# rhoposit/self-attention-tacotron

Hardware: AMD Instinct MI355X
Metric: teacher-forced mel frames/sec, LJSpeech batch=32, 1/2/4/8 MI355X (higher is better)
Workload: dtype fp32; 1 GPU; LJSpeech self-attention-tacotron.json teacher-forced training step (fwd + BPTT + Adam), configs[1]; global_batch=32, per_gpu_batch=32, chars=200, mel_frames=1000, num_mels=80, r=2, decoder_steps=500, parallelism=dp1, hip_graph=True, params=6227928

## Files before the change

include/sat_abi.h:

```cpp
#ifndef SAT_ABI_H
#define SAT_ABI_H

#include <stdint.h>

#ifdef __cplusplus
extern "C" {
#endif

#define SAT_OK 0
#define SAT_ERR_ARGUMENT -1
#define SAT_ERR_HIP -2
#define SAT_ERR_UNSUPPORTED -3

#define SAT_ABI_VERSION 11

int sat_version(void);
int sat_abi_version(void);
const char* sat_last_error_string(void);
int sat_device_arch(char* buf, int len);

typedef struct SatGemmDesc {
  int32_t M, N, K, batch;
  int32_t a_mode, a_L, a_C, a_shift;
  const float* A;
  int64_t a_sm, a_sk, a_sbatch;
  int32_t b_mode, b_taps, b_C, act;
  const float* B;
  int64_t b_sk, b_sn, b_sbatch;
  float* C;
// ... 288 lines not shown

typedef struct SatDecAttnFwd {
  int32_t B, N, T, U, M1, M2, D1, D2, F, KW;
  float u, zc, zh;
  const float* X0; const float* W0r; const float* Wq1; const float* Wq2;
  const float* K1; const float* V1; const float* K2; const float* V2;
  const int64_t* lengths;
  const float* v1; const float* b1; const float* convW; const float* convb; const float* locW;
  const float* v2;
  const float* mask_c; const float* mask_h;
  float* REC0; float* C0; float* H0RAW; float* G0; float* Q;
  float* S1; float* AL1; float* S2; float* ST; float* LOC;
  float* E; float* PART; float* QP; uint32_t* ctr; int32_t* err;
  int64_t* prof;
  float* ZH;
} SatDecAttnFwd;

int sat_decoder_attention_fwd(const SatDecAttnFwd* args, void* stream);
int64_t sat_decoder_attention_scratch(int32_t B, int32_t N, int64_t* e_floats, int64_t* part_floats,
                                      int64_t* qp_floats);

typedef struct SatDecAttnBwd {
  int32_t B, N, T, U, M1, M2, D1, D2, F, KW;
  float u, zc, zh;
  const float* REC0; const float* C0; const float* G0;
  const float* S1; const float* AL1; const float* S2; const float* ST; const float* LOC;
  const float* V1; const float* V2;
  const float* v1; const float* convW; const float* convb; const float* locW;
  const float* v2;
  const float* W0r; const float* Wq1; const float* Wq2;
// ... 199 lines not shown
```

self-attention-tacotron_amd/_lib.py:

```python

from __future__ import annotations

import ctypes
import os
from typing import Optional

PKG_DIR = os.path.dirname(os.path.abspath(__file__))
LIB_PATH = os.environ.get("SAT_LIB_OVERRIDE") or os.path.join(PKG_DIR, "libsat_hip.so")


class SatLibraryError(RuntimeError):

    def __init__(self, msg: str, rc: Optional[int] = None):
        super().__init__(msg)
        self.rc = rc


SAT_ERR_ARGUMENT = -1
SAT_ERR_UNSUPPORTED = -3


class SatGemmDesc(ctypes.Structure):
    _fields_ = [
        ("M", ctypes.c_int32), ("N", ctypes.c_int32), ("K", ctypes.c_int32),
# ... 91 lines not shown
SatAttnAgentBwd = _struct("SatAttnAgentBwd", """
    i32:B i32:ntiles i32:M1 i32:D1 i32:D2 ptr:dup ptr:u_t ptr:agent_w ptr:dz_out
    ptr:dctx i64:dctx_sb ptr:dq_extra i64:dq_sb""")

SatAttnParamGrad = _struct("SatAttnParamGrad", """
    i32:T i32:B i32:N i32:D1 i32:D2 i32:F i32:KW i32:att1_forward ptr:K1 ptr:K2
    ptr:q i64:q_tstride i64:q_bstride ptr:b1 ptr:v1 ptr:locW ptr:v2 ptr:loc
    ptr:s_prev i64:s_tstride ptr:de1 ptr:de2 ptr:df ptr:dK1 ptr:dK2 ptr:pg i64:pg_stride
    i32:tsplit""")

SatDecAttnFwd = _struct("SatDecAttnFwd", """
    i32:B i32:N i32:T i32:U i32:M1 i32:M2 i32:D1 i32:D2 i32:F i32:KW f32:u f32:zc f32:zh
    ptr:X0 ptr:W0r ptr:Wq1 ptr:Wq2 ptr:K1 ptr:V1 ptr:K2 ptr:V2 ptr:lengths
    ptr:v1 ptr:b1 ptr:convW ptr:convb ptr:locW ptr:v2 ptr:mask_c ptr:mask_h
    ptr:REC0 ptr:C0 ptr:H0RAW ptr:G0 ptr:Q ptr:S1 ptr:AL1 ptr:S2 ptr:ST ptr:LOC
    ptr:E ptr:PART ptr:QP ptr:ctr ptr:err ptr:prof ptr:ZH""")

SatDecAttnBwd = _struct("SatDecAttnBwd", """
    i32:B i32:N i32:T i32:U i32:M1 i32:M2 i32:D1 i32:D2 i32:F i32:KW f32:u f32:zc f32:zh
    ptr:REC0 ptr:C0 ptr:G0 ptr:S1 ptr:AL1 ptr:S2 ptr:ST ptr:LOC
    ptr:V1 ptr:V2 ptr:v1 ptr:convW ptr:convb ptr:locW ptr:v2
    ptr:W0r ptr:Wq1 ptr:Wq2 ptr:mask_c ptr:mask_h ptr:DH0 ptr:ZH
    ptr:RD ptr:DG0 ptr:DE1 ptr:DE2 ptr:DFH ptr:DQP ptr:RDP ptr:YA ptr:ctr ptr:err ptr:prof""")

SatDecLstmFwd = _struct("SatDecLstmFwd", """
    i32:B i32:T i32:U f32:zc f32:zh ptr:X1 ptr:W1r ptr:W2 ptr:b2
    ptr:mask1_c ptr:mask1_h ptr:mask2_c ptr:mask2_h
    ptr:H1RAW ptr:C1S ptr:H1S ptr:G1 ptr:H2RAW ptr:C2S ptr:H2S ptr:G2 ptr:xch ptr:err ptr:prof""")

SatDecLstmBwd = _struct("SatDecLstmBwd", """
    i32:B i32:T i32:U f32:zc f32:zh ptr:W1r ptr:W2 ptr:G1 ptr:C1S ptr:G2 ptr:C2S ptr:DH2
# ... 125 lines not shown
            "sat_mha_scratch_bytes": (ctypes.c_int64, [_I32, _I32, _I32, _I32, _I32]),
            "sat_mha_scratch_bytes_fused": (ctypes.c_int64, [_I32, _I32, _I32, _I32, _I32]),
            "sat_workspace_size": (ctypes.c_int64, [ctypes.c_void_p]),
            "sat_decoder_attention_scratch": (ctypes.c_int64, [_I32, _I32, _P, _P, _P]),
            "sat_decoder_attention_bwd_scratch": (ctypes.c_int64, [_I32, _I32, _P, _P]),
            "sat_decoder_attention_bwd_dq_parts": (ctypes.c_int32, [_I32, _I32]),
            "sat_decoder_lstms_scratch": (ctypes.c_int64, [_I32]),
            "sat_decode_persistent_scratch_bytes": (ctypes.c_int64, []),
            "sat_decoder_lstms_bwd_scratch": (ctypes.c_int64, [_I32]),
            "sat_crc32c": (ctypes.c_uint32, [_P, _I64, ctypes.c_uint32]),
            "sat_tfrecord_masked_crc": (ctypes.c_uint32, [_P, _I64]),
            "sat_tfrecord_frame": (ctypes.c_int64, [_P, _I64, _P]),
            "sat_tfrecord_index": (ctypes.c_int64, [_P, _I64, _I32, _P, _I64])}

_lib: Optional[ctypes.CDLL] = None
ABI_VERSION = 11


def load(path: str = LIB_PATH) -> ctypes.CDLL:
    global _lib
    if _lib is not None:
        return _lib
    if not os.path.exists(path):
        raise SatLibraryError(f"{path} not found: run __graft_entry__.build() (make -C csrc)")
    lib = ctypes.CDLL(path)
    got = lib.sat_abi_version() if hasattr(lib, "sat_abi_version") else None
    if got != ABI_VERSION:
        raise SatLibraryError(f"{path}: ABI version {got}, this binding needs {ABI_VERSION} "
                              "(rebuild it: make -C self-attention-tacotron_amd/csrc)")
    for name, argtypes in SIGNATURES.items():
        fn = getattr(lib, name)
# ... 48 lines not shown
```

self-attention-tacotron_amd/csrc/decoder_persistent8.hip:

```cpp
#include "sat_common.h"
#include "persistent.h"

#ifndef SAT_FWD8_TRACE
#define SAT_FWD8_TRACE 0
#endif
#ifndef SAT_FWD8_NORM3
#define SAT_FWD8_NORM3 1
#endif
#ifndef SAT_FWD8_HSTORE7
#define SAT_FWD8_HSTORE7 1
#endif
#ifndef SAT_FWD8_ESCALE
#define SAT_FWD8_ESCALE 1
#endif
#ifndef SAT_FWD8_POLL1
#define SAT_FWD8_POLL1 1
#endif
#ifndef SAT_FWD8_HMERGE
#define SAT_FWD8_HMERGE 1
#endif

#ifndef SAT_FWD8_R1
#define SAT_FWD8_R1 1
#endif
#ifndef SAT_FWD8_R2
#define SAT_FWD8_R2 1
#endif
#ifndef SAT_FWD8_STW
#define SAT_FWD8_STW 1
#endif
#ifndef SAT_FWD8_R4
#define SAT_FWD8_R4 0
#endif
#ifndef SAT_FWD8_C2W
#define SAT_FWD8_C2W 0
#endif

namespace sat {
namespace {

constexpr int kW = 8;
constexpr int kGmax = 32;
constexpr int kTh = 512;
constexpr int kU = 256, kM1 = 256, kM2 = 32, kD1 = 224, kD2 = 32, kF = 5, kKW = 10;
constexpr int kC = kM1 + kM2;
constexpr int kK0 = kC + kU;
constexpr int kQ = kD1 + kD2;
constexpr int kUW = kU / kW;
constexpr int kPmax = 32;
constexpr int kPadL = (kKW - 1) / 2;
constexpr int kPadR = kKW - 1 - kPadL;
constexpr int kRA = kQ + kUW;
constexpr int kRB = 320;
constexpr int kRBctx = 8, kRBeh = kRBctx + kC, kRBet = kRBeh + kPadR, kRBal = kRBet + kPadL;
constexpr int kR4 = 2 + kC / 4;
constexpr float kTwoLog2e = 2.8853900817779268f;
static_assert(kRBal + 2 <= kRB && kK0 == 544 && kQ == 256 && kD1 % 16 == 0, "layout");

struct Fwd8P {
  int B, N, T, P, flags;
  float u, zc, zh;
  const float* X0; const float* W0r; const float* Wq1; const float* Wq2;
  const float* K1; const float* V1; const float* K2; const float* V2;
  const int64_t* lengths;
  const float* v1; const float* b1; const float* convW; const float* convb; const float* locW;
  const float* v2;
  const float* mask_c; const float* mask_h;
  float* REC0; float* C0; float* H0RAW; float* G0; float* Q;
  float* S1; float* AL1; float* S2; float* ST; float* LOC; float* ZH;
  float* RA;
  float* RB;
  unsigned* XID;
  int* err;
  long long* prof;
};

typedef float f2 __attribute__((ext_vector_type(2)));
typedef float f4v __attribute__((ext_vector_type(4)));
// ... 6 lines not shown
  return make_float4(a.x + b.x, a.y + b.y, a.z + b.z, a.w + b.w);
}
__device__ __forceinline__ float sigm_fast(float x) {
  return __builtin_amdgcn_rcpf(1.f + __expf(-x));
}
__device__ __forceinline__ float fold32(float x) {
  const auto r = __builtin_amdgcn_permlane32_swap(__float_as_uint(x), __float_as_uint(x), false, false);
  return __uint_as_float(r[0]) + __uint_as_float(r[1]);
}
__device__ __forceinline__ float4 quad_gather(float x) {
  return make_float4(x, dpp_mov<0x101>(x), dpp_mov<0x102>(x), dpp_mov<0x103>(x));
}

__global__ void __launch_bounds__(kTh) dec_attn_fwd8_kernel(Fwd8P p) {
  __shared__ __attribute__((aligned(16))) float kc[kPmax][kQ];
  __shared__ __attribute__((aligned(16))) float v1s[kPmax][kM1];
  __shared__ __attribute__((aligned(16))) float v2s[kPmax][kM2];
  __shared__ __attribute__((aligned(16))) float wqs[kUW][kQ];
  __shared__ __attribute__((aligned(16))) float wc2[kM2][4 * kUW + 4];
  __shared__ __attribute__((aligned(16))) float cwl[kKW][kQ];
  __shared__ __attribute__((aligned(16))) float vcat[kQ];
  __shared__ float cw[kKW * kF + kF];
  __shared__ __attribute__((aligned(16))) float hbuf[kU];
  __shared__ __attribute__((aligned(16))) float cbuf[kC];
  __shared__ __attribute__((aligned(16))) float4 qst[kW][64];
  __shared__ __attribute__((aligned(16))) float4 recs[kW][kR4];
  __shared__ __attribute__((aligned(16))) float hst[kUW];
  __shared__ __attribute__((aligned(16))) float hraw[kUW];
  __shared__ float cown[kUW];
  __shared__ __attribute__((aligned(16))) float4 gown[kUW];
  __shared__ float gsum[8][64];
  __shared__ float halo[12];
  __shared__ float eown[kPmax], e2own[kPmax];
  __shared__ float alf[2][kPmax + 1];
  __shared__ float sp[kPmax + kKW];
  __shared__ __attribute__((aligned(16))) float wsc[8][2][kPmax];
  __shared__ long long tp[16];

  const int tid0 = threadIdx.x;
  const int g = blockIdx.x % kGmax, j = blockIdx.x / kGmax;
  const int B = p.B, N = p.N, T = p.T, P = p.P;
  if (g >= B) return;
  const int b = g;
  const int n0 = j * P, nt = max(0, min(P, N - n0));
  const bool has_left = j > 0, has_right = j + 1 < kW && n0 + P < N;
  const bool w7_stores = SAT_FWD8_HSTORE7 && 4 * 7 >= nt;
  const int64_t bN = (int64_t)b * N;
  const int len = (int)p.lengths[b];
  const float u = p.u;
  const auto rRA = rsrc(p.RA), rRB = rsrc(p.RB);

  f2 w0[8][8];
  {
    const int lane = tid0 & 63, wave = tid0 >> 6;
#pragma unroll
    for (int i = 0; i < 8; ++i) {
      const int r = i < 4 ? kC + 64 * i + lane : 64 * (i - 4) + lane;
      const float4* src = reinterpret_cast<const float4*>(p.W0r + (int64_t)r * (4 * kU) +
                                                          128 * j + 16 * wave);
#pragma unroll
      for (int q = 0; q < 4; ++q) {
        const float4 a = src[q];
        w0[i][2 * q] = f2{a.x, a.y};
        w0[i][2 * q + 1] = f2{a.z, a.w};
      }
    }
  }
  for (int i = tid0; i < kM2 * 32; i += kTh) {
    const int r = i >> 5, c4 = i & 31;
    *reinterpret_cast<float4*>(&wc2[r][4 * c4]) =
        reinterpret_cast<const float4*>(p.W0r + (int64_t)(kM1 + r) * (4 * kU) + 128 * j)[c4];
  }
  for (int i = tid0; i < kUW * kQ; i += kTh) {
    const int uu = i / kQ, c = i - uu * kQ, k = kUW * j + uu;
    wqs[uu][c] = c < kD1 ? p.Wq1[k * kD1 + c] : p.Wq2[k * kD2 + (c - kD1)];
  }
  for (int i = tid0; i < kPmax * kQ; i += kTh) {
// ... 3 lines not shown
#pragma unroll
      for (int f = 0; f < kF; ++f) lb = fmaf(p.convb[f], p.locW[f * kD1 + c], lb);
    }
    const float kv = r >= nt ? 0.f : c < kD1 ? p.K1[(bN + n0 + r) * kD1 + c] + p.b1[c] + lb
                                            : p.K2[(bN + n0 + r) * kD2 + (c - kD1)];
    kc[r][c] = SAT_FWD8_ESCALE ? kv * kTwoLog2e : kv;
  }
  for (int i = tid0; i < kKW * kQ; i += kTh) {
    const int k = i / kQ, c = i - k * kQ;
    float a = 0.f;
    if (c < kD1) {
#pragma unroll
      for (int f = 0; f < kF; ++f) a = fmaf(p.convW[k * kF + f], p.locW[f * kD1 + c], a);
    }
    cwl[k][c] = SAT_FWD8_ESCALE ? a * kTwoLog2e : a;
  }
  for (int i = tid0; i < kPmax * kM1 / 4; i += kTh) {
    const int r = i / (kM1 / 4), c4 = i - r * (kM1 / 4);
    reinterpret_cast<float4*>(&v1s[r][0])[c4] = r < nt
        ? reinterpret_cast<const float4*>(p.V1 + (bN + n0 + r) * kM1)[c4] : make_float4(0, 0, 0, 0);
  }
  for (int i = tid0; i < kPmax * kM2; i += kTh) {
    const int r = i / kM2, c = i - r * kM2;
    v2s[r][c] = r < nt ? p.V2[(bN + n0 + r) * kM2 + c] : 0.f;
  }
  for (int d = tid0; d < kQ; d += kTh) vcat[d] = d < kD1 ? p.v1[d] : p.v2[d - kD1];
  if (tid0 < kKW * kF) cw[tid0] = p.convW[tid0];
  if (tid0 < kF) cw[kKW * kF + tid0] = p.convb[tid0];
  if (tid0 < kU) hbuf[tid0] = 0.f;
  if (tid0 < 16) tp[tid0] = 0;
  gsum[tid0 >> 6][tid0 & 63] = 0.f;
  if (tid0 < nt + kKW - 1) {
    const int n = n0 - kPadL + tid0;
    sp[tid0] = (n >= 0 && n < N) ? p.S1[bN + n] : 0.f;
  }
// ... 86 lines not shown
      if (evt && t >= 100 && t < 108 && lane == 0) evt[((t - 100) * 8 + wave) * 16 + k] = wall_clock64();
      if (gevt && t >= 100 && t < 108 && tid == 0 && (k == 7 || k == 10 || k == 15 || k == 2)) {
        const int slot = k == 7 ? 0 : k == 10 ? 1 : k == 15 ? 2 : 3;
        const int ts = k == 2 ? t - 1 : t;
        if (ts >= 100) gevt[(ts - 100) * 32 + slot] = wall_clock64();
      }
#else
      (void)k;
#endif
    };
    ev(0);
    if (t > 0) {
      const int rb0 = ((s & 1) * B + b) * kW;
      const unsigned want = lsb_tag(s);
      const int rec = (rb0 + wave) * kRB;
      const bool two = lane < kM2 / 4 + 2;
      const int i2 = lane < kM2 / 4 ? (rec + kRBctx + kM1) / 4 + lane : rec / 4 + (lane - kM2 / 4);
      const int hq = lane - 16;
      const bool hl = wave == 0 && hq >= 0 && hq < 11;
      const bool hleft = hq < kPadL || hq >= kPadL + kPadR;
      const bool hsrc = hl && (hleft ? has_left : has_right);
      const int hw = (rb0 + (hleft ? j - 1 : j + 1)) * kRB +
                     (hq < kPadL ? kRBet + hq : hq < kPadL + kPadR ? kRBeh + hq - kPadL
                                                                   : kRBal + hq - kPadL - kPadR);
      float4 x1 = make_float4(0.f, 0.f, 0.f, 0.f), x2 = x1;
      float hv = 0.f;
      bool ok1 = false, ok2 = !two, ok3 = !hsrc;
#if SAT_FWD8_TRACE
      const long long tq0 = wall_clock64();
      asm volatile("s_waitcnt vmcnt(0)" ::: "memory");
      const long long tq1 = wall_clock64();
#endif
      bool retry = true;
      if (SAT_FWD8_POLL1) {
        x1 = ldc4(rRB, (rec + kRBctx) / 4 + lane);
        x2 = ldc4(rRB, i2);
        const float h0 = ldc(rRB, hsrc ? hw : 0);
        hv = hsrc ? h0 : 0.f;
        ok1 = tag_ok4(x1, want);
        ok2 = ok2 || tag_ok4(x2, want);
        ok3 = ok3 || tag_ok(hv, want);
        retry = any_lane(!(ok1 && ok2 && ok3)) && !gave_up;
      }
      if (retry) {
        for (unsigned spins = 0;; ++spins) {
          if (!ok1) x1 = ldc4(rRB, (rec + kRBctx) / 4 + lane);
          if (!ok2) x2 = ldc4(rRB, i2);
          if (!ok3) hv = ldc(rRB, hsrc ? hw : 0);
          ok1 = tag_ok4(x1, want);
          ok2 = ok2 || tag_ok4(x2, want);
          ok3 = ok3 || tag_ok(hv, want);
          if (!any_lane(!(ok1 && ok2 && ok3)) || gave_up) break;
          if (poll_give_up(spins, p.err)) { gave_up = true; break; }
          __builtin_amdgcn_s_sleep(1);
        }
      }
#if SAT_FWD8_TRACE
      {
        const long long tq2 = wall_clock64();
        if (evt && t >= 100 && t < 108 && lane == 0) {
          evt[8 * 8 * 16 + ((t - 100) * 8 + wave) * 4 + 0] = tq1 - tq0;
          evt[8 * 8 * 16 + ((t - 100) * 8 + wave) * 4 + 1] = tq2 - tq1;
        }
      }
#endif
      recs[wave][2 + lane] = x1;
      if (lane < kM2 / 4) recs[wave][2 + kM1 / 4 + lane] = x2;
      else if (two) recs[wave][lane - kM2 / 4] = x2;
      if (hl) halo[hq] = hv;
      tick(0);
    ev(1);
      lds_barrier();
      tick(1);
    ev(2);
      {
        const int jj = lane & 7;
        const float4 st = recs[jj][0];
        const float z2 = recs[jj][1].x;
        M1 = lanes8_max(st.x);
        M2 = lanes8_max(st.w);
        const float sc1 = __expf(st.x - M1), sc2 = __expf(st.w - M2);
        Z1 = lanes8_sum(st.y * sc1);
        A1 = lanes8_sum(st.z * sc1);
        Z2 = lanes8_sum(z2 * sc2);
        if (wave < (kC + 63) / 64) {
          if (tid < kC) {
            const bool first = wave < kM1 / 64;
            const float sc = first ? sc1 : sc2;
            const float* rf = reinterpret_cast<const float*>(&recs[0][2]) + tid;
            float a = 0.f;
#pragma unroll
            for (int k = 0; k < kW; ++k) a = fmaf(rf[k * kR4 * 4], rdl(sc, k), a);
            a *= __builtin_amdgcn_rcpf(first ? A1 : Z2);
            cbuf[tid] = a;
            if (tid / (kC / kW) == j) p.REC0[((int64_t)t * B + b) * kK0 + tid] = a;
          }
        } else {
          const unsigned bit = lsb_tag(t);
          if (wave == 5) {
            if (lane < nt + kKW - 1) {
              const float e = e_at(n0 - kPadL + lane);
              const float sv = e == -INFINITY ? 0.f : __expf(e - M1) * __builtin_amdgcn_rcpf(Z1);
              sp[lane] = sv;
              if (!SAT_FWD8_NORM3 && lane >= kPadL && lane < nt + kPadL)
                p.S1[((int64_t)t * B + b) * N + n0 + lane - kPadL] = sv;
            }
            if (t < T && 4 * 7 < nt) {
              asm volatile("s_waitcnt lgkmcnt(0)" ::: "memory");
              store_loc(t, lane);
            }
// ... 44 lines not shown
      f2 acc[8];
#pragma unroll
      for (int q = 0; q < 8; ++q) acc[q] = f2{0.f, 0.f};
      if (t > 0) {
#if SAT_FWD8_HMERGE
#pragma unroll
        for (int i = 0; i < 4; ++i) {
          const float xv = hbuf[64 * i + lane];
          const f2 xx = {xv, xv};
#pragma unroll
          for (int q = 0; q < 8; ++q) acc[q] = __builtin_elementwise_fma(xx, w0[i][q], acc[q]);
        }
#endif
#pragma unroll
        for (int i = 4; i < 8; ++i) {
          const float xv = cbuf[64 * (i - 4) + lane];
          const f2 xx = {xv, xv};
#pragma unroll
          for (int q = 0; q < 8; ++q) acc[q] = __builtin_elementwise_fma(xx, w0[i][q], acc[q]);
        }
        const int r2 = lane & 31, hsel = lane >> 5;
        const float xv = cbuf[kM1 + r2];
        const f2 xx = {xv, xv};
        const float4 wa = *reinterpret_cast<const float4*>(&wc2[r2][16 * wave + 8 * hsel]);
        const float4 wb = *reinterpret_cast<const float4*>(&wc2[r2][16 * wave + 8 * hsel + 4]);
        const f2 c0 = __builtin_elementwise_fma(xx, f2{wa.x, wa.y}, f2{0.f, 0.f});
        const f2 c1 = __builtin_elementwise_fma(xx, f2{wa.z, wa.w}, f2{0.f, 0.f});
        const f2 c2 = __builtin_elementwise_fma(xx, f2{wb.x, wb.y}, f2{0.f, 0.f});
        const f2 c3 = __builtin_elementwise_fma(xx, f2{wb.z, wb.w}, f2{0.f, 0.f});
        if (hsel == 0) { acc[0] += c0; acc[1] += c1; acc[2] += c2; acc[3] += c3; }
        else { acc[4] += c0; acc[5] += c1; acc[6] += c2; acc[7] += c3; }
      }
      float v[16];
#pragma unroll
      for (int q = 0; q < 8; ++q) { v[2 * q] = acc[q].x; v[2 * q + 1] = acc[q].y; }
      transpose_reduce16(v, lane);
      const int gate = (lane >> 2) & 3;
// ... 189 lines not shown
          p.C0[((int64_t)(t + 1) * B + b) * kU + cunit] = cown[lane];
          p.REC0[((int64_t)(t + 1) * B + b) * kK0 + kC + cunit] = hst[lane];
          p.H0RAW[tbu] = hraw[lane];
          reinterpret_cast<float4*>(p.G0)[tbu] = gown[lane];
        }
      }
    }
    tick(11);
    ev(12);
    lds_barrier();
    tick(12);
    ev(13);
    {
      const unsigned bit = lsb_tag(t);
      const float* al = alf[t & 1];
      if (SAT_FWD8_R2 && wave == 7 && lane < kPadR + kPadL + 2) {
        const int rb = (((t & 1) * B + b) * kW + j) * kRB;
        const int q = lane;
        float v;
        if (q < kPadR) v = q < nt ? eown[q] : -INFINITY;
        else if (q < kPadR + kPadL) { const int i = nt - kPadL + (q - kPadR); v = i >= 0 ? eown[i] : -INFINITY; }
        else { const int k = nt - 1 + (q - kPadR - kPadL); v = k >= 0 ? al[k] : 0.f; }
        stcx(xl, rRB, rb + kRBeh + q, tagf(v == -INFINITY ? 0.f : v, bit));
      }
      const float e1v = lane < kPmax ? eown[lane] : -INFINITY;
      const float e2v = lane < kPmax ? e2own[lane] : -INFINITY;
      const float m1 = tagf(fmaxf(wave_max_dpp(e1v), -3.402823466e38f), bit);
      const float m2 = tagf(fmaxf(wave_max_dpp(e2v), -3.402823466e38f), bit);
      const float pe = e1v == -INFINITY ? 0.f : __expf(e1v - m1);
      const float pe2 = e2v == -INFINITY ? 0.f : __expf(e2v - m2);
      const float w = lane < nt ? ((1.f - u) * al[lane + 1] + u * al[lane] + 1e-7f) * pe : 0.f;
      if (lane < kPmax) { wsc[wave][0][lane] = w; wsc[wave][1][lane] = lane < nt ? pe2 : 0.f; }
      if (wave == SAT_FWD8_STW) {
        const float z1 = tagf(wave_sum_dpp(pe), bit), a1 = tagf(wave_sum_dpp(w), bit);
        const float z2 = tagf(wave_sum_dpp(pe2), bit);
        if (lane == 0) {
          const int rb = (((t & 1) * B + b) * kW + j) * kRB;
          stc4x(xl, rRB, rb / 4, make_float4(m1, z1, a1, m2));
          stc4x(xl, rRB, rb / 4 + 1, tagf4(make_float4(z2, 0.f, 0.f, 0.f), bit));
        }
      }
      asm volatile("s_waitcnt lgkmcnt(0)" ::: "memory");
    }
    tick(13);
    ev(14);
    {
      const unsigned bit = lsb_tag(t);
      const int rb = (((t & 1) * B + b) * kW + j) * kRB;
      const int col = lane & 31, r0 = 16 * (lane >> 5);
      const float* ws = &wsc[wave][0][r0];
      float c = 0.f;
#pragma unroll
      for (int k4 = 0; k4 < 4; ++k4) {
        const float4 w4 = *reinterpret_cast<const float4*>(ws + 4 * k4);
        c = fmaf(w4.x, v1s[r0 + 4 * k4][32 * wave + col], c);
        c = fmaf(w4.y, v1s[r0 + 4 * k4 + 1][32 * wave + col], c);
        c = fmaf(w4.z, v1s[r0 + 4 * k4 + 2][32 * wave + col], c);
        c = fmaf(w4.w, v1s[r0 + 4 * k4 + 3][32 * wave + col], c);
      }
      const float4 c4 = quad_gather(fold32(c));
      if (lane < 32 && (lane & 3) == 0)
        stc4x(xl, rRB, (rb + kRBctx) / 4 + 8 * wave + (lane >> 2), tagf4(c4, bit));
      if (wave == SAT_FWD8_C2W) {
        const float* ws2 = &wsc[SAT_FWD8_C2W][1][r0];
        float c2 = 0.f;
#pragma unroll
        for (int k = 0; k < 16; ++k) c2 = fmaf(ws2[k], v2s[r0 + k][col], c2);
        const float4 q4 = quad_gather(fold32(c2));
        if (lane < 32 && (lane & 3) == 0)
          stc4x(xl, rRB, (rb + kRBctx + kM1) / 4 + (lane >> 2), tagf4(q4, bit));
      } else if (!SAT_FWD8_R2 && wave == 1 && lane < kPadR + kPadL + 2) {
        const int q = lane;
        float v;
        if (q < kPadR) v = q < nt ? eown[q] : -INFINITY;
        else if (q < kPadR + kPadL) { const int i = nt - kPadL + (q - kPadR); v = i >= 0 ? eown[i] : -INFINITY; }
        else { const int k = nt - 1 + (q - kPadR - kPadL); v = k >= 0 ? alf[t & 1][k] : 0.f; }
        stcx(xl, rRB, rb + kRBeh + q, tagf(v == -INFINITY ? 0.f : v, bit));
      }
    }
    tick(14);
    ev(15);
    if (!SAT_FWD8_HMERGE && t + 1 < T) {
      f2 acc[8];
#pragma unroll
      for (int q = 0; q < 8; ++q) acc[q] = f2{0.f, 0.f};
#pragma unroll
      for (int i = 0; i < 4; ++i) {
        const float xv = hbuf[64 * i + lane];
        const f2 xx = {xv, xv};
#pragma unroll
        for (int q = 0; q < 8; ++q) acc[q] = __builtin_elementwise_fma(xx, w0[i][q], acc[q]);
      }
      float v[16];
#pragma unroll
// ... 6 lines not shown
#if SAT_FWD8_TRACE || SAT_SEGMENT_CLOCKS
  if (p.prof && tid0 == 0)
    for (int i = 0; i < 16; ++i) p.prof[blockIdx.x * 16 + i] = tp[i];
#endif
}

}

bool dec_attn_fwd8_eligible(const SatDecAttnFwd* a) {
  return a->U == kU && a->M1 == kM1 && a->M2 == kM2 && a->D1 == kD1 && a->D2 == kD2 &&
         a->F == kF && a->KW == kKW && a->B >= 1 && a->B <= kGmax && a->N >= 1 &&
         a->N <= kW * kPmax;
}

int dec_attn_fwd8_launch(const SatDecAttnFwd* a, hipStream_t s) {
  int dev = 0, cus = 0, per_cu = 0;
  if (hipGetDevice(&dev) != hipSuccess ||
      hipDeviceGetAttribute(&cus, hipDeviceAttributeMultiprocessorCount, dev) != hipSuccess ||
      hipOccupancyMaxActiveBlocksPerMultiprocessor(&per_cu, dec_attn_fwd8_kernel, kTh, 0) != hipSuccess) {
    set_error("sat_decoder_attention_fwd: device query failed");
    return SAT_ERR_HIP;
  }
  SAT_CHECK_ARG((int64_t)cus * per_cu >= kGmax * kW,
                "sat_decoder_attention_fwd: fewer than 256 co-resident workgroups on this device");
  Fwd8P p;
  p.B = a->B; p.N = a->N; p.T = a->T;
  p.P = std::max(kPadR, ceil_div(a->N, kW));
  p.u = a->u; p.zc = a->zc; p.zh = a->zh;
  p.X0 = a->X0; p.W0r = a->W0r; p.Wq1 = a->Wq1; p.Wq2 = a->Wq2;
  p.K1 = a->K1; p.V1 = a->V1; p.K2 = a->K2; p.V2 = a->V2; p.lengths = a->lengths;
  p.v1 = a->v1; p.b1 = a->b1; p.convW = a->convW; p.convb = a->convb; p.locW = a->locW;
  p.v2 = a->v2; p.mask_c = a->mask_c; p.mask_h = a->mask_h;
  p.REC0 = a->REC0; p.C0 = a->C0; p.H0RAW = a->H0RAW; p.G0 = a->G0; p.Q = a->Q;
  p.S1 = a->S1; p.AL1 = a->AL1; p.S2 = a->S2; p.ST = a->ST; p.LOC = a->LOC; p.ZH = a->ZH;
  const int64_t ra = (int64_t)2 * a->B * kW * kRA, rb = (int64_t)2 * a->B * kW * kRB;
  p.RA = a->QP;
  p.RB = a->QP + ra;
  p.XID = reinterpret_cast<unsigned*>(a->QP + ra + rb);
  p.err = a->err;
  p.flags = xcd_local_env();
  p.prof = reinterpret_cast<long long*>(a->prof);
  if (zero_ranges(s, a->QP, ra + rb + kGmax * kW, a->err, 2) != hipSuccess) {
    set_error("sat_decoder_attention_fwd: scratch clear failed");
    return SAT_ERR_HIP;
  }
  hipLaunchKernelGGL(dec_attn_fwd8_kernel, dim3(kGmax * kW), dim3(kTh), 0, s, p);
  SAT_LAUNCH_CHECK("sat_decoder_attention_fwd");
  return SAT_OK;
}

}
```

self-attention-tacotron_amd/decoder.py:

```python

from __future__ import annotations

import warnings
from dataclasses import dataclass, field
from typing import Dict, Optional

import torch

from . import kernels as K
from .params import Dims
from .pipeline import SEQUENTIAL, Pipeline


@dataclass
class DecoderSaved:
    B: int
    N: int
    Tp: int
    tensors: Dict[str, torch.Tensor] = field(default_factory=dict)

    def __getattr__(self, k):
        t = self.__dict__.get("tensors", {})
        if k in t:
            return t[k]
# ... 249 lines not shown
        n = (b - a) * B
        K.linear(L1[0][a:b].reshape(n, Dd), W2[:Dd], P["decoder/lstm2/bias"],
                 out=X2[a:b].view(n, 4 * Dd))

    def lstm1_desc(t):
        return _lstm_desc(X1, W1r, t, B, Dd, zc, zh, m1c, m1h, L1)

    def lstm2_desc(t):
        return _lstm_desc(X2, W2[Dd:], t, B, Dd, zc, zh, m2c, m2h, L2)

    if use_persistent(d, B, N, attn_tile, persistent):
        if scratch is None:
            scratch = K.DecoderAttentionScratch(B, N, dev)
        ZH = torch.empty(Tp, B, N, D1 + D2, **f32) if keep_tanh else None
        S["ZH"] = ZH
        K.decoder_attention_fwd(
            B=B, N=N, T=Tp, U=A, M1=M1, M2=M2, D1=D1, D2=D2, F=d.loc_f, KW=d.loc_k, u=0.5,
            zc=zc, zh=zh, X0=X0, W0r=Wr0, Wq1=P[f"{a1}/query_layer/kernel"],
            Wq2=P["decoder/attention2/query_layer/kernel"], K1=K1, V1=V1, K2=K2, V2=V2,
            lengths=lengths, v1=P[f"{a1}/attention_variable"], b1=P[f"{a1}/attention_bias"],
            convW=P[f"{a1}/location_conv/kernel"], convb=P[f"{a1}/location_conv/bias"],
            locW=P[f"{a1}/location_layer/kernel"], v2=P["decoder/attention2/attention_v"],
            mask_c=zc0, mask_h=zh0, REC0=REC0, C0=C0, H0RAW=H0RAW, G0=G0, Q=Q, S1=S1, AL1=AL1,
            S2=S2, ST=ST, LOC=LOC, E=scratch.E, PART=scratch.PART, QP=scratch.QP, ctr=scratch.ctr,
            err=scratch.err, ZH=ZH)
        S["attn_scratch"] = scratch
        x1_chunk(0, Tp)
        X2 = None
        K.decoder_lstms_fwd(
            B=B, T=Tp, U=Dd, zc=zc, zh=zh, X1=X1, W1r=W1r, W2=W2,
            b2=P["decoder/lstm2/bias"], mask1_c=m1c, mask1_h=m1h, mask2_c=m2c, mask2_h=m2h,
            H1RAW=L1[0], C1S=L1[1], H1S=L1[2], G1=L1[3], H2RAW=L2[0], C2S=L2[1], H2S=L2[2],
            G2=L2[3], xch=scratch.lstm_xch, err=scratch.lstm_err[0])
    elif not pipe.enabled:
        for t in range(Tp):
            K.lstm_step_fwd(**lstm0_desc(t))
            attention_rest(t)
        x1_chunk(0, Tp)
        for t in range(Tp):
            K.lstm_step_fwd(**lstm1_desc(t))
# ... 45 lines not shown
```

self-attention-tacotron_amd/kernels.py:

```python

from __future__ import annotations

import ctypes
import os

import torch

from . import _lib

ACT = {None: 0, "none": 0, "relu": 1, "tanh": 2, "sigmoid": 3, "softsign": 4}


def _stream() -> int:
    return torch.cuda.current_stream().cuda_stream


def _p(t) -> int:
    return 0 if t is None else t.data_ptr()


_GEMM_WS = {}
GEMM_WS_BYTES = 32 << 20


# ... 580 lines not shown
        self.lstm_ctr = torch.zeros(int(_lib.load().sat_decoder_lstms_bwd_scratch(B)),
                                    dtype=torch.int32, device=device)
        self.lstm_err = errs[2:6].view(2, 2)

    def check(self):
        if int(self.err[0].item()) != 0:
            raise _lib.SatLibraryError("sat_decoder_attention_fwd: an in-kernel hand-off timed out "
                                       "(workgroups not co-resident?)")
        for i, nm in enumerate(("sat_decoder_lstms_fwd", "sat_decoder_lstms_bwd")):
            if int(self.lstm_err[i, 0].item()) != 0:
                raise _lib.SatLibraryError(f"{nm}: a group barrier timed out "
                                           "(workgroups not co-resident?)")
        self.bwd.check()


def decoder_attention_fwd(**kw):
    a = _lib.SatDecAttnFwd()
    for k, v in kw.items():
        setattr(a, k, _p(v) if isinstance(v, torch.Tensor) else v)
    _lib.check(_lib.load().sat_decoder_attention_fwd(ctypes.byref(a), _stream()),
               "sat_decoder_attention_fwd")


class DecoderAttentionBwdScratch:

    def __init__(self, B: int, N: int, device, err: torch.Tensor = None):
        rdp, ya = ctypes.c_int64(), ctypes.c_int64()
        words = int(_lib.load().sat_decoder_attention_bwd_scratch(B, N, ctypes.byref(rdp),
                                                                  ctypes.byref(ya)))
        self.RDP = torch.empty(rdp.value, device=device)
# ... 342 lines not shown
```

Measured before the change: 2.429 million frames/s.

## Fold attention-1 values into LSTM weights and defer context GEMM off the recurrence

Precomputes VW1 = V1 @ W0r (the encoder values projected through the LSTM0 input weights) with a GEMM before the persistent decoder attention kernel. Each step then feeds the normalized per-position attention weights directly into the gate accumulation instead of first building the attention-1 context vector. The context vectors themselves are produced afterwards by a batched GEMM of the alignments with V1, outside the serial recurrence. This shrinks the cross-workgroup record, removes the per-step context reduction, and drops the v1s shared buffer, at the cost of two extra GEMMs and a B*N*4U scratch buffer. The first-step context row is written in-kernel while later rows come from the post-GEMM, so correctness depends on that offset split.

```diff
diff --git a/include/sat_abi.h b/include/sat_abi.h
--- a/include/sat_abi.h
+++ b/include/sat_abi.h
@@ -12,7 +12,7 @@
 #define SAT_ERR_HIP -2
 #define SAT_ERR_UNSUPPORTED -3
 
-#define SAT_ABI_VERSION 11
+#define SAT_ABI_VERSION 12
 
 int sat_version(void);
 int sat_abi_version(void);
@@ -331,6 +331,7 @@
   float* E; float* PART; float* QP; uint32_t* ctr; int32_t* err;
   int64_t* prof;
   float* ZH;
+  float* VW1;
 } SatDecAttnFwd;
 
 int sat_decoder_attention_fwd(const SatDecAttnFwd* args, void* stream);
diff --git a/self-attention-tacotron_amd/_lib.py b/self-attention-tacotron_amd/_lib.py
--- a/self-attention-tacotron_amd/_lib.py
+++ b/self-attention-tacotron_amd/_lib.py
@@ -129,7 +129,7 @@
     ptr:X0 ptr:W0r ptr:Wq1 ptr:Wq2 ptr:K1 ptr:V1 ptr:K2 ptr:V2 ptr:lengths
     ptr:v1 ptr:b1 ptr:convW ptr:convb ptr:locW ptr:v2 ptr:mask_c ptr:mask_h
     ptr:REC0 ptr:C0 ptr:H0RAW ptr:G0 ptr:Q ptr:S1 ptr:AL1 ptr:S2 ptr:ST ptr:LOC
-    ptr:E ptr:PART ptr:QP ptr:ctr ptr:err ptr:prof ptr:ZH""")
+    ptr:E ptr:PART ptr:QP ptr:ctr ptr:err ptr:prof ptr:ZH ptr:VW1""")
 
 SatDecAttnBwd = _struct("SatDecAttnBwd", """
     i32:B i32:N i32:T i32:U i32:M1 i32:M2 i32:D1 i32:D2 i32:F i32:KW f32:u f32:zc f32:zh
@@ -285,7 +285,7 @@
             "sat_tfrecord_index": (ctypes.c_int64, [_P, _I64, _I32, _P, _I64])}
 
 _lib: Optional[ctypes.CDLL] = None
-ABI_VERSION = 11
+ABI_VERSION = 12
 
 
 def load(path: str = LIB_PATH) -> ctypes.CDLL:
diff --git a/self-attention-tacotron_amd/csrc/decoder_persistent8.hip b/self-attention-tacotron_amd/csrc/decoder_persistent8.hip
--- a/self-attention-tacotron_amd/csrc/decoder_persistent8.hip
+++ b/self-attention-tacotron_amd/csrc/decoder_persistent8.hip
@@ -23,9 +23,6 @@
 #ifndef SAT_FWD8_R1
 #define SAT_FWD8_R1 1
 #endif
-#ifndef SAT_FWD8_R2
-#define SAT_FWD8_R2 1
-#endif
 #ifndef SAT_FWD8_STW
 #define SAT_FWD8_STW 1
 #endif
@@ -35,6 +32,8 @@
 #ifndef SAT_FWD8_C2W
 #define SAT_FWD8_C2W 0
 #endif
+static_assert(SAT_FWD8_STW != SAT_FWD8_C2W && SAT_FWD8_STW != 7 && SAT_FWD8_C2W != 7,
+              "record B's publishers are three different waves");
 
 namespace sat {
 namespace {
@@ -51,17 +50,19 @@
 constexpr int kPadL = (kKW - 1) / 2;
 constexpr int kPadR = kKW - 1 - kPadL;
 constexpr int kRA = kQ + kUW;
-constexpr int kRB = 320;
-constexpr int kRBctx = 8, kRBeh = kRBctx + kC, kRBet = kRBeh + kPadR, kRBal = kRBet + kPadL;
-constexpr int kR4 = 2 + kC / 4;
+constexpr int kRB = 96;
+constexpr int kRBw = 8, kRBc2 = kRBw + kPmax, kRBeh = kRBc2 + kM2, kRBet = kRBeh + kPadR;
+constexpr int kRBal = kRBet + kPadL;
+constexpr int kR4 = 2 + kPmax / 4 + kM2 / 4;
 constexpr float kTwoLog2e = 2.8853900817779268f;
-static_assert(kRBal + 2 <= kRB && kK0 == 544 && kQ == 256 && kD1 % 16 == 0, "layout");
+static_assert(kRBal + 2 <= kRB && kRB % 4 == 0 && kK0 == 544 && kQ == 256 && kD1 % 16 == 0 &&
+              kW * kPmax == kM1, "layout");
 
 struct Fwd8P {
   int B, N, T, P, flags;
   float u, zc, zh;
   const float* X0; const float* W0r; const float* Wq1; const float* Wq2;
-  const float* K1; const float* V1; const float* K2; const float* V2;
+  const float* K1; const float* VW1; const float* K2; const float* V2;
   const int64_t* lengths;
   const float* v1; const float* b1; const float* convW; const float* convb; const float* locW;
   const float* v2;
@@ -98,7 +99,6 @@
 
 __global__ void __launch_bounds__(kTh) dec_attn_fwd8_kernel(Fwd8P p) {
   __shared__ __attribute__((aligned(16))) float kc[kPmax][kQ];
-  __shared__ __attribute__((aligned(16))) float v1s[kPmax][kM1];
   __shared__ __attribute__((aligned(16))) float v2s[kPmax][kM2];
   __shared__ __attribute__((aligned(16))) float wqs[kUW][kQ];
   __shared__ __attribute__((aligned(16))) float wc2[kM2][4 * kUW + 4];
@@ -106,7 +106,8 @@
   __shared__ __attribute__((aligned(16))) float vcat[kQ];
   __shared__ float cw[kKW * kF + kF];
   __shared__ __attribute__((aligned(16))) float hbuf[kU];
-  __shared__ __attribute__((aligned(16))) float cbuf[kC];
+  __shared__ __attribute__((aligned(16))) float abuf[kW * kPmax];
+  __shared__ __attribute__((aligned(16))) float c2buf[kM2];
   __shared__ __attribute__((aligned(16))) float4 qst[kW][64];
   __shared__ __attribute__((aligned(16))) float4 recs[kW][kR4];
   __shared__ __attribute__((aligned(16))) float hst[kUW];
@@ -118,7 +119,7 @@
   __shared__ float eown[kPmax], e2own[kPmax];
   __shared__ float alf[2][kPmax + 1];
   __shared__ float sp[kPmax + kKW];
-  __shared__ __attribute__((aligned(16))) float wsc[8][2][kPmax];
+  __shared__ __attribute__((aligned(16))) float w2s[kPmax];
   __shared__ long long tp[16];
 
   const int tid0 = threadIdx.x;
@@ -139,12 +140,14 @@
     const int lane = tid0 & 63, wave = tid0 >> 6;
 #pragma unroll
     for (int i = 0; i < 8; ++i) {
-      const int r = i < 4 ? kC + 64 * i + lane : 64 * (i - 4) + lane;
-      const float4* src = reinterpret_cast<const float4*>(p.W0r + (int64_t)r * (4 * kU) +
-                                                          128 * j + 16 * wave);
+      const int slot = 64 * (i - 4) + lane, sk = slot & (kPmax - 1), sn = (slot >> 5) * P + sk;
+      const bool live = i < 4 || (sk < P && sn < N);
+      const float* row = i < 4 ? p.W0r + (int64_t)(kC + 64 * i + lane) * (4 * kU)
+                               : p.VW1 + (bN + (live ? sn : 0)) * (4 * kU);
+      const float4* src = reinterpret_cast<const float4*>(row + 128 * j + 16 * wave);
 #pragma unroll
       for (int q = 0; q < 4; ++q) {
-        const float4 a = src[q];
+        const float4 a = live ? src[q] : make_float4(0.f, 0.f, 0.f, 0.f);
         w0[i][2 * q] = f2{a.x, a.y};
         w0[i][2 * q + 1] = f2{a.z, a.w};
       }
@@ -178,11 +181,6 @@
       for (int f = 0; f < kF; ++f) a = fmaf(p.convW[k * kF + f], p.locW[f * kD1 + c], a);
     }
     cwl[k][c] = SAT_FWD8_ESCALE ? a * kTwoLog2e : a;
-  }
-  for (int i = tid0; i < kPmax * kM1 / 4; i += kTh) {
-    const int r = i / (kM1 / 4), c4 = i - r * (kM1 / 4);
-    reinterpret_cast<float4*>(&v1s[r][0])[c4] = r < nt
-        ? reinterpret_cast<const float4*>(p.V1 + (bN + n0 + r) * kM1)[c4] : make_float4(0, 0, 0, 0);
   }
   for (int i = tid0; i < kPmax * kM2; i += kTh) {
     const int r = i / kM2, c = i - r * kM2;
@@ -299,8 +297,8 @@
       const int rb0 = ((s & 1) * B + b) * kW;
       const unsigned want = lsb_tag(s);
       const int rec = (rb0 + wave) * kRB;
-      const bool two = lane < kM2 / 4 + 2;
-      const int i2 = lane < kM2 / 4 ? (rec + kRBctx + kM1) / 4 + lane : rec / 4 + (lane - kM2 / 4);
+      const bool one = lane < kR4;
+      const int q1 = lane < kR4 - 2 ? 2 + lane : one ? lane - (kR4 - 2) : 0;
       const int hq = lane - 16;
       const bool hl = wave == 0 && hq >= 0 && hq < 11;
       const bool hleft = hq < kPadL || hq >= kPadL + kPadR;
@@ -308,9 +306,9 @@
       const int hw = (rb0 + (hleft ? j - 1 : j + 1)) * kRB +
                      (hq < kPadL ? kRBet + hq : hq < kPadL + kPadR ? kRBeh + hq - kPadL
                                                                    : kRBal + hq - kPadL - kPadR);
-      float4 x1 = make_float4(0.f, 0.f, 0.f, 0.f), x2 = x1;
+      float4 x1 = make_float4(0.f, 0.f, 0.f, 0.f);
       float hv = 0.f;
-      bool ok1 = false, ok2 = !two, ok3 = !hsrc;
+      bool ok1 = !one, ok3 = !hsrc;
 #if SAT_FWD8_TRACE
       const long long tq0 = wall_clock64();
       asm volatile("s_waitcnt vmcnt(0)" ::: "memory");
@@ -318,24 +316,20 @@
 #endif
       bool retry = true;
       if (SAT_FWD8_POLL1) {
-        x1 = ldc4(rRB, (rec + kRBctx) / 4 + lane);
-        x2 = ldc4(rRB, i2);
+        x1 = ldc4(rRB, rec / 4 + q1);
         const float h0 = ldc(rRB, hsrc ? hw : 0);
         hv = hsrc ? h0 : 0.f;
-        ok1 = tag_ok4(x1, want);
-        ok2 = ok2 || tag_ok4(x2, want);
+        ok1 = ok1 || tag_ok4(x1, want);
         ok3 = ok3 || tag_ok(hv, want);
-        retry = any_lane(!(ok1 && ok2 && ok3)) && !gave_up;
+        retry = any_lane(!(ok1 && ok3)) && !gave_up;
       }
       if (retry) {
         for (unsigned spins = 0;; ++spins) {
-          if (!ok1) x1 = ldc4(rRB, (rec + kRBctx) / 4 + lane);
-          if (!ok2) x2 = ldc4(rRB, i2);
+          if (!ok1) x1 = ldc4(rRB, rec / 4 + q1);
           if (!ok3) hv = ldc(rRB, hsrc ? hw : 0);
-          ok1 = tag_ok4(x1, want);
-          ok2 = ok2 || tag_ok4(x2, want);
+          ok1 = ok1 || tag_ok4(x1, want);
           ok3 = ok3 || tag_ok(hv, want);
-          if (!any_lane(!(ok1 && ok2 && ok3)) || gave_up) break;
+          if (!any_lane(!(ok1 && ok3)) || gave_up) break;
           if (poll_give_up(spins, p.err)) { gave_up = true; break; }
           __builtin_amdgcn_s_sleep(1);
         }
@@ -349,9 +343,7 @@
         }
       }
 #endif
-      recs[wave][2 + lane] = x1;
-      if (lane < kM2 / 4) recs[wave][2 + kM1 / 4 + lane] = x2;
-      else if (two) recs[wave][lane - kM2 / 4] = x2;
+      if (one) recs[wave][q1] = x1;
       if (hl) halo[hq] = hv;
       tick(0);
     ev(1);
@@ -368,17 +360,19 @@
         Z1 = lanes8_sum(st.y * sc1);
         A1 = lanes8_sum(st.z * sc1);
         Z2 = lanes8_sum(z2 * sc2);
-        if (wave < (kC + 63) / 64) {
-          if (tid < kC) {
-            const bool first = wave < kM1 / 64;
-            const float sc = first ? sc1 : sc2;
-            const float* rf = reinterpret_cast<const float*>(&recs[0][2]) + tid;
+        if (wave < kM1 / 64) {
+          const float s_lo = rdl(sc1, 2 * wave), s_hi = rdl(sc1, 2 * wave + 1);
+          const float wv = reinterpret_cast<const float*>(&recs[tid >> 5][2])[lane & (kPmax - 1)];
+          abuf[tid] = wv * (lane < 32 ? s_lo : s_hi) * __builtin_amdgcn_rcpf(A1);
+        } else if (wave == kM1 / 64) {
+          if (lane < kM2) {
+            const float* rf = reinterpret_cast<const float*>(&recs[0][2 + kPmax / 4]) + lane;
             float a = 0.f;
 #pragma unroll
-            for (int k = 0; k < kW; ++k) a = fmaf(rf[k * kR4 * 4], rdl(sc, k), a);
-            a *= __builtin_amdgcn_rcpf(first ? A1 : Z2);
-            cbuf[tid] = a;
-            if (tid / (kC / kW) == j) p.REC0[((int64_t)t * B + b) * kK0 + tid] = a;
+            for (int k = 0; k < kW; ++k) a = fmaf(rf[k * kR4 * 4], rdl(sc2, k), a);
+            a *= __builtin_amdgcn_rcpf(Z2);
+            c2buf[lane] = a;
+            if (lane / (kM2 / kW) == j) p.REC0[((int64_t)t * B + b) * kK0 + kM1 + lane] = a;
           }
         } else {
           const unsigned bit = lsb_tag(t);
@@ -453,13 +447,13 @@
 #endif
 #pragma unroll
         for (int i = 4; i < 8; ++i) {
-          const float xv = cbuf[64 * (i - 4) + lane];
+          const float xv = abuf[64 * (i - 4) + lane];
           const f2 xx = {xv, xv};
 #pragma unroll
           for (int q = 0; q < 8; ++q) acc[q] = __builtin_elementwise_fma(xx, w0[i][q], acc[q]);
         }
         const int r2 = lane & 31, hsel = lane >> 5;
-        const float xv = cbuf[kM1 + r2];
+        const float xv = c2buf[r2];
         const f2 xx = {xv, xv};
         const float4 wa = *reinterpret_cast<const float4*>(&wc2[r2][16 * wave + 8 * hsel]);
         const float4 wb = *reinterpret_cast<const float4*>(&wc2[r2][16 * wave + 8 * hsel + 4]);
@@ -679,70 +673,50 @@
     {
       const unsigned bit = lsb_tag(t);
       const float* al = alf[t & 1];
-      if (SAT_FWD8_R2 && wave == 7 && lane < kPadR + kPadL + 2) {
-        const int rb = (((t & 1) * B + b) * kW + j) * kRB;
-        const int q = lane;
-        float v;
-        if (q < kPadR) v = q < nt ? eown[q] : -INFINITY;
-        else if (q < kPadR + kPadL) { const int i = nt - kPadL + (q - kPadR); v = i >= 0 ? eown[i] : -INFINITY; }
-        else { const int k = nt - 1 + (q - kPadR - kPadL); v = k >= 0 ? al[k] : 0.f; }
-        stcx(xl, rRB, rb + kRBeh + q, tagf(v == -INFINITY ? 0.f : v, bit));
-      }
-      const float e1v = lane < kPmax ? eown[lane] : -INFINITY;
-      const float e2v = lane < kPmax ? e2own[lane] : -INFINITY;
-      const float m1 = tagf(fmaxf(wave_max_dpp(e1v), -3.402823466e38f), bit);
-      const float m2 = tagf(fmaxf(wave_max_dpp(e2v), -3.402823466e38f), bit);
-      const float pe = e1v == -INFINITY ? 0.f : __expf(e1v - m1);
-      const float pe2 = e2v == -INFINITY ? 0.f : __expf(e2v - m2);
-      const float w = lane < nt ? ((1.f - u) * al[lane + 1] + u * al[lane] + 1e-7f) * pe : 0.f;
-      if (lane < kPmax) { wsc[wave][0][lane] = w; wsc[wave][1][lane] = lane < nt ? pe2 : 0.f; }
-      if (wave == SAT_FWD8_STW) {
+      const int rb = (((t & 1) * B + b) * kW + j) * kRB;
+      if (wave == 7) {
+        if (lane < kPadR + kPadL + 2) {
+          const int q = lane;
+          float v;
+          if (q < kPadR) v = q < nt ? eown[q] : -INFINITY;
+          else if (q < kPadR + kPadL) { const int i = nt - kPadL + (q - kPadR); v = i >= 0 ? eown[i] : -INFINITY; }
+          else { const int k = nt - 1 + (q - kPadR - kPadL); v = k >= 0 ? al[k] : 0.f; }
+          stcx(xl, rRB, rb + kRBeh + q, tagf(v == -INFINITY ? 0.f : v, bit));
+        }
+      } else if (wave == SAT_FWD8_STW) {
+        const float e1v = lane < kPmax ? eown[lane] : -INFINITY;
+        const float e2v = lane < kPmax ? e2own[lane] : -INFINITY;
+        const float m1 = tagf(fmaxf(wave_max_dpp(e1v), -3.402823466e38f), bit);
+        const float m2 = tagf(fmaxf(wave_max_dpp(e2v), -3.402823466e38f), bit);
+        const float pe = e1v == -INFINITY ? 0.f : __expf(e1v - m1);
+        const float pe2 = e2v == -INFINITY ? 0.f : __expf(e2v - m2);
+        const float w = lane < nt ? ((1.f - u) * al[lane + 1] + u * al[lane] + 1e-7f) * pe : 0.f;
         const float z1 = tagf(wave_sum_dpp(pe), bit), a1 = tagf(wave_sum_dpp(w), bit);
         const float z2 = tagf(wave_sum_dpp(pe2), bit);
+        const float4 w4 = quad_gather(w);
+        if (lane < kPmax && (lane & 3) == 0)
+          stc4x(xl, rRB, (rb + kRBw) / 4 + (lane >> 2), tagf4(w4, bit));
         if (lane == 0) {
-          const int rb = (((t & 1) * B + b) * kW + j) * kRB;
           stc4x(xl, rRB, rb / 4, make_float4(m1, z1, a1, m2));
           stc4x(xl, rRB, rb / 4 + 1, tagf4(make_float4(z2, 0.f, 0.f, 0.f), bit));
         }
-      }
-      asm volatile("s_waitcnt lgkmcnt(0)" ::: "memory");
+      } else if (wave == SAT_FWD8_C2W) {
+        const float e2v = lane < kPmax ? e2own[lane] : -INFINITY;
+        const float m2 = tagf(fmaxf(wave_max_dpp(e2v), -3.402823466e38f), bit);
+        const float pe2 = e2v == -INFINITY ? 0.f : __expf(e2v - m2);
+        if (lane < kPmax) w2s[lane] = lane < nt ? pe2 : 0.f;
+        asm volatile("s_waitcnt lgkmcnt(0)" ::: "memory");
+        const int col = lane & 31, r0 = 16 * (lane >> 5);
+        float c2 = 0.f;
+#pragma unroll
+        for (int k = 0; k < 16; ++k) c2 = fmaf(w2s[r0 + k], v2s[r0 + k][col], c2);
+        const float4 q4 = quad_gather(fold32(c2));
+        if (lane < 32 && (lane & 3) == 0)
+          stc4x(xl, rRB, (rb + kRBc2) / 4 + (lane >> 2), tagf4(q4, bit));
+      }
     }
     tick(13);
     ev(14);
-    {
-      const unsigned bit = lsb_tag(t);
-      const int rb = (((t & 1) * B + b) * kW + j) * kRB;
-      const int col = lane & 31, r0 = 16 * (lane >> 5);
-      const float* ws = &wsc[wave][0][r0];
-      float c = 0.f;
-#pragma unroll
-      for (int k4 = 0; k4 < 4; ++k4) {
-        const float4 w4 = *reinterpret_cast<const float4*>(ws + 4 * k4);
-        c = fmaf(w4.x, v1s[r0 + 4 * k4][32 * wave + col], c);
-        c = fmaf(w4.y, v1s[r0 + 4 * k4 + 1][32 * wave + col], c);
-        c = fmaf(w4.z, v1s[r0 + 4 * k4 + 2][32 * wave + col], c);
-        c = fmaf(w4.w, v1s[r0 + 4 * k4 + 3][32 * wave + col], c);
-      }
-      const float4 c4 = quad_gather(fold32(c));
-      if (lane < 32 && (lane & 3) == 0)
-        stc4x(xl, rRB, (rb + kRBctx) / 4 + 8 * wave + (lane >> 2), tagf4(c4, bit));
-      if (wave == SAT_FWD8_C2W) {
-        const float* ws2 = &wsc[SAT_FWD8_C2W][1][r0];
-        float c2 = 0.f;
-#pragma unroll
-        for (int k = 0; k < 16; ++k) c2 = fmaf(ws2[k], v2s[r0 + k][col], c2);
-        const float4 q4 = quad_gather(fold32(c2));
-        if (lane < 32 && (lane & 3) == 0)
-          stc4x(xl, rRB, (rb + kRBctx + kM1) / 4 + (lane >> 2), tagf4(q4, bit));
-      } else if (!SAT_FWD8_R2 && wave == 1 && lane < kPadR + kPadL + 2) {
-        const int q = lane;
-        float v;
-        if (q < kPadR) v = q < nt ? eown[q] : -INFINITY;
-        else if (q < kPadR + kPadL) { const int i = nt - kPadL + (q - kPadR); v = i >= 0 ? eown[i] : -INFINITY; }
-        else { const int k = nt - 1 + (q - kPadR - kPadL); v = k >= 0 ? alf[t & 1][k] : 0.f; }
-        stcx(xl, rRB, rb + kRBeh + q, tagf(v == -INFINITY ? 0.f : v, bit));
-      }
-    }
     tick(14);
     ev(15);
     if (!SAT_FWD8_HMERGE && t + 1 < T) {
@@ -779,6 +753,9 @@
 }
 
 int dec_attn_fwd8_launch(const SatDecAttnFwd* a, hipStream_t s) {
+  SAT_CHECK_ARG(a->VW1 && aligned16(a->VW1),
+                "sat_decoder_attention_fwd: VW1 [B][N][4U] (16-byte aligned) is required for "
+                "N <= 256");
   int dev = 0, cus = 0, per_cu = 0;
   if (hipGetDevice(&dev) != hipSuccess ||
       hipDeviceGetAttribute(&cus, hipDeviceAttributeMultiprocessorCount, dev) != hipSuccess ||
@@ -793,7 +770,7 @@
   p.P = std::max(kPadR, ceil_div(a->N, kW));
   p.u = a->u; p.zc = a->zc; p.zh = a->zh;
   p.X0 = a->X0; p.W0r = a->W0r; p.Wq1 = a->Wq1; p.Wq2 = a->Wq2;
-  p.K1 = a->K1; p.V1 = a->V1; p.K2 = a->K2; p.V2 = a->V2; p.lengths = a->lengths;
+  p.K1 = a->K1; p.VW1 = a->VW1; p.K2 = a->K2; p.V2 = a->V2; p.lengths = a->lengths;
   p.v1 = a->v1; p.b1 = a->b1; p.convW = a->convW; p.convb = a->convb; p.locW = a->locW;
   p.v2 = a->v2; p.mask_c = a->mask_c; p.mask_h = a->mask_h;
   p.REC0 = a->REC0; p.C0 = a->C0; p.H0RAW = a->H0RAW; p.G0 = a->G0; p.Q = a->Q;
@@ -809,9 +786,25 @@
     set_error("sat_decoder_attention_fwd: scratch clear failed");
     return SAT_ERR_HIP;
   }
+  SatGemmDesc d;
+  std::memset(&d, 0, sizeof(d));
+  d.M = a->B * a->N; d.N = 4 * kU; d.K = kM1; d.batch = 1; d.batch2 = 1;
+  d.A = a->V1; d.a_sm = kM1; d.a_sk = 1;
+  d.B = a->W0r; d.b_sk = 4 * kU; d.b_sn = 1;
+  d.C = a->VW1; d.c_sm = 4 * kU;
+  d.alpha = 1.f; d.beta = 0.f;
+  int rc = sat_gemm(&d, s);
+  if (rc != SAT_OK) return rc;
   hipLaunchKernelGGL(dec_attn_fwd8_kernel, dim3(kGmax * kW), dim3(kTh), 0, s, p);
   SAT_LAUNCH_CHECK("sat_decoder_attention_fwd");
-  return SAT_OK;
-}
-
-}
+  std::memset(&d, 0, sizeof(d));
+  d.M = a->T; d.N = kM1; d.K = a->N; d.batch = a->B; d.batch2 = 1;
+  d.A = a->AL1 + (int64_t)a->B * a->N; d.a_sm = (int64_t)a->B * a->N; d.a_sk = 1;
+  d.a_sbatch = a->N;
+  d.B = a->V1; d.b_sk = kM1; d.b_sn = 1; d.b_sbatch = (int64_t)a->N * kM1;
+  d.C = a->REC0 + (int64_t)a->B * kK0; d.c_sm = (int64_t)a->B * kK0; d.c_sbatch = kK0;
+  d.alpha = 1.f; d.beta = 0.f;
+  return sat_gemm(&d, s);
+}
+
+}
diff --git a/self-attention-tacotron_amd/decoder.py b/self-attention-tacotron_amd/decoder.py
--- a/self-attention-tacotron_amd/decoder.py
+++ b/self-attention-tacotron_amd/decoder.py
@@ -287,6 +287,8 @@
             scratch = K.DecoderAttentionScratch(B, N, dev)
         ZH = torch.empty(Tp, B, N, D1 + D2, **f32) if keep_tanh else None
         S["ZH"] = ZH
+        VW1 = torch.empty(B, N, 4 * A, **f32) if K.decoder_attention_takes_vw1(N) else None
+        S["VW1"] = VW1
         K.decoder_attention_fwd(
             B=B, N=N, T=Tp, U=A, M1=M1, M2=M2, D1=D1, D2=D2, F=d.loc_f, KW=d.loc_k, u=0.5,
             zc=zc, zh=zh, X0=X0, W0r=Wr0, Wq1=P[f"{a1}/query_layer/kernel"],
@@ -296,7 +298,7 @@
             locW=P[f"{a1}/location_layer/kernel"], v2=P["decoder/attention2/attention_v"],
             mask_c=zc0, mask_h=zh0, REC0=REC0, C0=C0, H0RAW=H0RAW, G0=G0, Q=Q, S1=S1, AL1=AL1,
             S2=S2, ST=ST, LOC=LOC, E=scratch.E, PART=scratch.PART, QP=scratch.QP, ctr=scratch.ctr,
-            err=scratch.err, ZH=ZH)
+            err=scratch.err, ZH=ZH, VW1=VW1)
         S["attn_scratch"] = scratch
         x1_chunk(0, Tp)
         X2 = None
diff --git a/self-attention-tacotron_amd/kernels.py b/self-attention-tacotron_amd/kernels.py
--- a/self-attention-tacotron_amd/kernels.py
+++ b/self-attention-tacotron_amd/kernels.py
@@ -618,6 +618,10 @@
         self.bwd.check()
 
 
+def decoder_attention_takes_vw1(N: int) -> bool:
+    return N <= 256
+
+
 def decoder_attention_fwd(**kw):
     a = _lib.SatDecAttnFwd()
     for k, v in kw.items():
```

Result: no change. 2.441 million frames/s (median of 6 runs) (+0.5%).
